# ZhangHaoyang493/News_Recsys

Measured on AMD Instinct MI355X. Metric: impressions/sec at batch 65536 (embedding hot path forward), higher is better.
Workload: dtype f32

## Files before the change

news_recsys_amd/csrc/nrx_interact.hip:

```cpp
#include "nrx_common.h"

namespace {

__global__ __launch_bounds__(NRX_BLOCK) void bag_pool_fwd_kernel(const float* __restrict__ emb, const float* __restrict__ mask,
                                                                 int64_t batch, int L, int D, float* __restrict__ out) {
    const int64_t total = batch * (int64_t)D;
    for (int64_t i = (int64_t)blockIdx.x * NRX_BLOCK + threadIdx.x; i < total; i += (int64_t)gridDim.x * NRX_BLOCK) {
        const int64_t b = i / D;
        const int d = (int)(i - b * D);
        const float* e = emb + (b * L) * (int64_t)D + d;
        float acc = 0.f, den = 0.f;
        if (mask != nullptr) {
            const float* m = mask + b * (int64_t)L;
            for (int l = 0; l < L; ++l) {
#pragma clang fp contract(off)
                const float w = m[l];
                den += w;
                acc += e[(int64_t)l * D] * w;
            }
            out[i] = acc / (den + 1e-8f);
        } else {
            for (int l = 0; l < L; ++l) acc += e[(int64_t)l * D];
            out[i] = acc / (float)L;
        }
    }
}

template <bool VEC>
__global__ __launch_bounds__(NRX_BLOCK) void bag_pool_bwd_kernel(const float* __restrict__ g_out, const float* __restrict__ mask,
                                                                 int64_t batch, int L, int D, float* __restrict__ g_emb) {
    const int lane = threadIdx.x & 63;
    const int64_t wave = (int64_t)blockIdx.x * (NRX_BLOCK / 64) + (threadIdx.x >> 6);
    const int64_t nwaves = (int64_t)gridDim.x * (NRX_BLOCK / 64);
    const int n = L * D;
    for (int64_t b = wave; b < batch; b += nwaves) {
        float den = (float)L;
        if (mask != nullptr) {
            float part = 0.f;
            for (int l = lane; l < L; l += NRX_WAVE) part += mask[b * (int64_t)L + l];
            den = nrx_wave_sum(part) + 1e-8f;
        }
        const float* gb = g_out + b * (int64_t)D;
        const float* mb = mask ? mask + b * (int64_t)L : nullptr;
        float* ob = g_emb + b * (int64_t)n;
        if (VEC) {
            const unsigned q = (unsigned)D >> 2;
            for (unsigned e4 = lane; e4 < (unsigned)n >> 2; e4 += NRX_WAVE) {
                const unsigned l = e4 / q, d = (e4 - l * q) * 4;
                const float4 g = *reinterpret_cast<const float4*>(gb + d);
                const float m = mb ? mb[l] : 1.0f;
                float4 o = make_float4(g.x / den, g.y / den, g.z / den, g.w / den);
                if (mb) o = make_float4(o.x * m, o.y * m, o.z * m, o.w * m);
                *reinterpret_cast<float4*>(ob + (size_t)e4 * 4) = o;
            }
        } else {
            for (int e = lane; e < n; e += NRX_WAVE) {
                const int l = e / D, d = e - l * D;
                const float g = gb[d] / den;
                ob[e] = mb ? g * mb[l] : g;
            }
        }
    }
}

__device__ __forceinline__ float4 ld4(const float* p, int k0, int D, bool vec) {
    float4 v;
    if (vec) {
        v = *reinterpret_cast<const float4*>(p);
    } else {
        v.x = p[0];
        v.y = (k0 + 1 < D) ? p[1] : 0.f;
        v.z = (k0 + 2 < D) ? p[2] : 0.f;
        v.w = (k0 + 3 < D) ? p[3] : 0.f;
    }
    return v;
}

template <int QLOG2>
__global__ __launch_bounds__(NRX_BLOCK) void fm_fwd_kernel(const float* __restrict__ feat, int64_t ld, int F, int D,
                                                           int64_t batch, float* __restrict__ fm_out, bool vec,
                                                           float* __restrict__ sums = nullptr, int64_t sums_ld = 0) {
    constexpr int Q = 1 << QLOG2;
    constexpr int TB = NRX_BLOCK / Q;
    const int q = threadIdx.x & (Q - 1);
    const int64_t b = (int64_t)blockIdx.x * TB + (threadIdx.x >> QLOG2);
    const bool live = b < batch;
    float total = 0.f;
    for (int kc = 0; kc < D; kc += 4 * Q) {
        const int k0 = kc + q * 4;
        float first = 0.f;
        float4 s = make_float4(0.f, 0.f, 0.f, 0.f), sq = s;
        if (live && k0 < D) {
            const float* row = feat + b * ld + k0;
            for (int f = 0; f < F; ++f) {
                float4 v = ld4(row + (int64_t)f * D, k0, D, vec);
                if (k0 == 0) { first += v.x; v.x = 0.f; }
                s.x += v.x; s.y += v.y; s.z += v.z; s.w += v.w;
                sq.x += v.x * v.x; sq.y += v.y * v.y; sq.z += v.z * v.z; sq.w += v.w * v.w;
            }
        }
        total += 0.5f * ((s.x * s.x - sq.x) + (s.y * s.y - sq.y) + (s.z * s.z - sq.z) + (s.w * s.w - sq.w)) + first;
        if (sums != nullptr && live && k0 < D) {
            float* dst = sums + b * sums_ld + k0;
            const float v0 = k0 == 0 ? first : s.x;
            dst[0] = v0;
            if (k0 + 1 < D) dst[1] = s.y;
            if (k0 + 2 < D) dst[2] = s.z;
            if (k0 + 3 < D) dst[3] = s.w;
        }
    }
#pragma unroll
    for (int off = Q / 2; off > 0; off >>= 1) total += __shfl_xor(total, off, 64);
    if (live && q == 0) fm_out[b] = total;
}

template <int QLOG2>
__global__ __launch_bounds__(NRX_BLOCK) void fm_bwd_kernel(const float* __restrict__ feat, int64_t ld, int F, int D, int64_t batch,
                                                           const float* __restrict__ g_fm, const float* g_in, int64_t g_in_ld,
                                                           float* g_feat, int64_t g_ld, bool vec) {
    constexpr int Q = 1 << QLOG2;
    constexpr int TB = NRX_BLOCK / Q;
    constexpr int U = 8;
    const int q = threadIdx.x & (Q - 1);
    const int64_t b = (int64_t)blockIdx.x * TB + (threadIdx.x >> QLOG2);
    if (b >= batch) return;
    const float gl = g_fm[b];
    const bool gvec = vec && (g_ld & 3) == 0 && ((reinterpret_cast<uintptr_t>(g_feat) & 15u) == 0) &&
                      (g_in == nullptr || ((g_in_ld & 3) == 0 && (reinterpret_cast<uintptr_t>(g_in) & 15u) == 0));
    for (int kc = 0; kc < D; kc += 4 * Q) {
        const int k0 = kc + q * 4;
        if (k0 >= D) continue;
        const float* row = feat + b * ld + k0;
        const float* irow = g_in ? g_in + b * g_in_ld + k0 : nullptr;
        float* grow = g_feat + b * g_ld + k0;
        float4 s = make_float4(0.f, 0.f, 0.f, 0.f);
        int f = 0;
        for (; f + U <= F; f += U) {
            float4 v[U];
#pragma unroll
            for (int u = 0; u < U; ++u) v[u] = ld4(row + (int64_t)(f + u) * D, k0, D, vec);
#pragma unroll
            for (int u = 0; u < U; ++u) { s.x += v[u].x; s.y += v[u].y; s.z += v[u].z; s.w += v[u].w; }
        }
        for (; f < F; ++f) {
            const float4 v = ld4(row + (int64_t)f * D, k0, D, vec);
            s.x += v.x; s.y += v.y; s.z += v.z; s.w += v.w;
        }
        f = 0;
        if (gvec && k0 + 4 <= D) {
            for (; f + U <= F; f += U) {
                float4 v[U], up[U];
#pragma unroll
                for (int u = 0; u < U; ++u) {
                    v[u] = ld4(row + (int64_t)(f + u) * D, k0, D, vec);
                    up[u] = irow ? *reinterpret_cast<const float4*>(irow + (int64_t)(f + u) * D) : make_float4(0.f, 0.f, 0.f, 0.f);
                }
#pragma unroll
                for (int u = 0; u < U; ++u) {
                    float4 g = make_float4(gl * (s.x - v[u].x), gl * (s.y - v[u].y), gl * (s.z - v[u].z), gl * (s.w - v[u].w));
                    if (k0 == 0) g.x = gl;
                    *reinterpret_cast<float4*>(grow + (int64_t)(f + u) * D) = make_float4(up[u].x + g.x, up[u].y + g.y, up[u].z + g.z, up[u].w + g.w);
                }
            }
        }
        for (; f < F; ++f) {
            const float4 v = ld4(row + (int64_t)f * D, k0, D, vec);
            float g[4] = {gl * (s.x - v.x), gl * (s.y - v.y), gl * (s.z - v.z), gl * (s.w - v.w)};
            if (k0 == 0) g[0] = gl;
            float* gp = grow + (int64_t)f * D;
            const float* ip = irow ? irow + (int64_t)f * D : nullptr;
#pragma unroll
            for (int j = 0; j < 4; ++j)
                if (k0 + j < D) gp[j] = (ip ? ip[j] : 0.f) + g[j];
        }
    }
}

template <int R, int V>
struct RowRegs {
    float v[R][V];
};

template <int R, int V>
__device__ __forceinline__ void row_load(RowRegs<R, V>& x, const float* p, int D, int lane) {
#pragma unroll
    for (int r = 0; r < R; ++r) {
        const int c = (r * 64 + lane) * V;
        if (V == 4) {
            float4 t = make_float4(0.f, 0.f, 0.f, 0.f);
            if (c < D) t = *reinterpret_cast<const float4*>(p + c);
            x.v[r][0] = t.x; x.v[r][1 % V] = t.y; x.v[r][2 % V] = t.z; x.v[r][3 % V] = t.w;
        } else {
            x.v[r][0] = (c < D) ? p[c] : 0.f;
        }
    }
}

template <int R, int V>
__device__ __forceinline__ void row_store(const RowRegs<R, V>& x, float* p, int D, int lane) {
#pragma unroll
    for (int r = 0; r < R; ++r) {
        const int c = (r * 64 + lane) * V;
        if (c < D) {
            if (V == 4) *reinterpret_cast<float4*>(p + c) = make_float4(x.v[r][0], x.v[r][1 % V], x.v[r][2 % V], x.v[r][3 % V]);
            else p[c] = x.v[r][0];
        }
    }
}

__device__ __forceinline__ float nrx_half_wave_sum(float v, bool upper) {
    v += nrx_dpp<0xB1>(v);
    v += nrx_dpp<0x4E>(v);
    v += nrx_dpp<0x141>(v);
    v += nrx_dpp<0x140>(v);
    const float r0 = __builtin_bit_cast(float, __builtin_amdgcn_readlane(__builtin_bit_cast(int, v), 0));
    const float r1 = __builtin_bit_cast(float, __builtin_amdgcn_readlane(__builtin_bit_cast(int, v), 16));
    const float r2 = __builtin_bit_cast(float, __builtin_amdgcn_readlane(__builtin_bit_cast(int, v), 32));
    const float r3 = __builtin_bit_cast(float, __builtin_amdgcn_readlane(__builtin_bit_cast(int, v), 48));
    return upper ? r2 + r3 : r0 + r1;
}

template <int R, int V, int G = 64>
__device__ __forceinline__ float row_dot(const RowRegs<R, V>& a, const RowRegs<R, V>& b, bool upper = false) {
    float s = 0.f;
#pragma unroll
    for (int r = 0; r < R; ++r)
#pragma unroll
        for (int j = 0; j < V; ++j) s += a.v[r][j] * b.v[r][j];
    return G == 64 ? nrx_wave_sum(s) : nrx_half_wave_sum(s, upper);
}

template <int R, int V, int G = 64>
__global__ __launch_bounds__(NRX_BLOCK) void dcn_v1_fwd_kernel(const float* __restrict__ x, int64_t x_ld, const float* __restrict__ x0p,
                                                               int64_t x0_ld, int64_t batch, int D, int NL,
                                                               const float* __restrict__ w, const float* __restrict__ bvec,
                                                               float* __restrict__ out, int64_t out_ld) {
    extern __shared__ __attribute__((aligned(16))) char smem[];
    float* s_w = reinterpret_cast<float*>(smem);
    const int Dp = (D + 3) & ~3;
    float* s_b = s_w + NL * Dp;
    for (int i = threadIdx.x; i < NL * Dp; i += NRX_BLOCK) {
        const int l = i / Dp, c = i - l * Dp;
        s_w[i] = (c < D) ? w[l * (int64_t)D + c] : 0.f;
        s_b[i] = (c < D) ? bvec[l * (int64_t)D + c] : 0.f;
    }
    __syncthreads();
    constexpr int RPW = 64 / G;
    const int lane = threadIdx.x & (G - 1);
    const bool upper = G == 32 && (threadIdx.x & 32) != 0;
    const int64_t wave = (int64_t)blockIdx.x * (NRX_BLOCK / 64) + (threadIdx.x >> 6);
    const int64_t nwaves = (int64_t)gridDim.x * (NRX_BLOCK / 64);
    for (int64_t r0 = wave * RPW; r0 < batch; r0 += nwaves * RPW) {
        const int64_t rr = r0 + (upper ? 1 : 0);
        const bool live = rr < batch;
        const int64_t row = live ? rr : batch - 1;
        RowRegs<R, V> x0, xl;
        row_load<R, V>(xl, x + row * x_ld, D, lane);
        if (x0p != nullptr) row_load<R, V>(x0, x0p + row * x0_ld, D, lane);
        else x0 = xl;
        for (int l = 0; l < NL; ++l) {
            RowRegs<R, V> wl, bl;
            row_load<R, V>(wl, s_w + l * Dp, Dp, lane);
            row_load<R, V>(bl, s_b + l * Dp, Dp, lane);
            const float s = row_dot<R, V, G>(xl, wl, upper);
#pragma unroll
            for (int r = 0; r < R; ++r)
// ... 386 lines not shown
    const NRX_CONST EmbedDcnArgs* a = nrx_kernarg<EmbedDcnArgs>();
    constexpr int Q = 1 << QLOG2;
    constexpr int TB = NRX_BLOCK / Q;
    extern __shared__ __attribute__((aligned(16))) char smem[];
    const int W = a->width, NL = a->n_layers;
    float4* s_w = reinterpret_cast<float4*>(smem);
    float4* s_b = s_w + NL * (W / 4);
    const int q = threadIdx.x & (Q - 1);
    const int64_t batch = a->batch, stride = (int64_t)gridDim.x * TB;
    int64_t b = (int64_t)blockIdx.x * TB + (threadIdx.x >> QLOG2);
    auto load_ids = [&](int64_t bb, int64_t (&id)[N]) {
        const int64_t bc = bb < batch ? bb : batch - 1;
#pragma unroll
        for (int u = 0; u < N; ++u)
            id[u] = IDX64 ? nrx_gconst<int64_t>(a->index[u])[bc] : (int64_t)nrx_gconst<int32_t>(a->index[u])[bc];
    };
    int64_t id[N];
    load_ids(b, id);
    for (int i = threadIdx.x; i < NL * (W / 4); i += NRX_BLOCK) {
        s_w[i] = reinterpret_cast<const float4*>(a->w)[i];
        s_b[i] = reinterpret_cast<const float4*>(a->b)[i];
    }
    __syncthreads();
    for (; b - (threadIdx.x >> QLOG2) < batch; b += stride) {
        const bool live = b < batch;
        float4 x0[N];
        int bad_feat = -1;
        int64_t bad_id = 0;
#pragma unroll
        for (int u = 0; u < N; ++u) {
            const bool bad = (uint64_t)id[u] >= (uint64_t)a->rows[u];
            bad_feat = bad ? u : bad_feat;
            bad_id = bad ? id[u] : bad_id;
            x0[u] = NT ? nrx_ldg4_nt(a->table[u], (bad ? 0 : id[u]) * Q + q) : nrx_ldg4(a->table[u], (bad ? 0 : id[u]) * Q + q);
        }
        if (bad_feat >= 0 && q == 0 && live) nrx_report_oob(a->status, bad_feat, b, bad_id);
        if (b - (threadIdx.x >> QLOG2) + stride < batch) load_ids(b + stride, id);
        if (EARLY && live) {
            NRX_GLOBAL nrx_f32x4* o = (NRX_GLOBAL nrx_f32x4*)(a->out + b * a->out_ld);
#pragma unroll
            for (int u = 0; u < N; ++u) {
                nrx_f32x4 t;
                t.x = x0[u].x; t.y = x0[u].y; t.z = x0[u].z; t.w = x0[u].w;
                if (STNT) __builtin_nontemporal_store(t, o + u * Q + q);
                else o[u * Q + q] = t;
            }
        }
        float4 xl[N];
#pragma unroll
        for (int u = 0; u < N; ++u) xl[u] = x0[u];
        for (int l = 0; l < NL; ++l) {
            const float4* wl = s_w + l * (W / 4) + q;
            const float4* bl = s_b + l * (W / 4) + q;
            float part = 0.f;
#pragma unroll
            for (int u = 0; u < N; ++u) {
                const float4 wv = wl[u * Q];
                part += xl[u].x * wv.x + xl[u].y * wv.y + xl[u].z * wv.z + xl[u].w * wv.w;
            }
            const float dot = group_sum_dpp<Q>(part);
#pragma unroll
            for (int u = 0; u < N; ++u) {
                const float4 bv = bl[u * Q];
                xl[u].x = x0[u].x * dot + bv.x + xl[u].x;
                xl[u].y = x0[u].y * dot + bv.y + xl[u].y;
                xl[u].z = x0[u].z * dot + bv.z + xl[u].z;
                xl[u].w = x0[u].w * dot + bv.w + xl[u].w;
            }
        }
        if (live) {
            NRX_GLOBAL nrx_f32x4* o = (NRX_GLOBAL nrx_f32x4*)(a->out + b * a->out_ld);
#pragma unroll
            for (int u = EARLY ? N : 0; u < 2 * N; ++u) {
                const float4 v = u < N ? x0[u] : xl[u - N];
                nrx_f32x4 t;
                t.x = v.x; t.y = v.y; t.z = v.z; t.w = v.w;
                NRX_GLOBAL nrx_f32x4* dst = o + (u < N ? 0 : W / 4) + (u < N ? u : u - N) * Q + q;
                if (STNT) __builtin_nontemporal_store(t, dst);
                else *dst = t;
            }
        }
    }
}

int ceil_log2i(int x) {
    int l = 0;
    while ((1 << l) < x) ++l;
    return l;
}

unsigned stream_grid(int64_t items, int per_block) {
    int64_t g = (items + per_block - 1) / per_block;
    const int64_t cap = 256 * 8;
    if (g > cap) g = cap;
    if (g < 1) g = 1;
    return (unsigned)g;
}

#define NRX_QSWITCH(qlog2, ...)               \
    switch (qlog2) {                           \
        case 0: { constexpr int QL = 0; __VA_ARGS__; } break; \
        case 1: { constexpr int QL = 1; __VA_ARGS__; } break; \
        case 2: { constexpr int QL = 2; __VA_ARGS__; } break; \
        case 3: { constexpr int QL = 3; __VA_ARGS__; } break; \
        case 4: { constexpr int QL = 4; __VA_ARGS__; } break; \
        case 5: { constexpr int QL = 5; __VA_ARGS__; } break; \
        default: { constexpr int QL = 6; __VA_ARGS__; } break; \
    }

#define NRX_RSWITCH(R_, V_, ...)                                   \
    if (V_ == 4) {                                                  \
        constexpr int VV = 4;                                       \
        if (R_ <= 1) { constexpr int RR = 1; __VA_ARGS__; }                \
        else if (R_ <= 2) { constexpr int RR = 2; __VA_ARGS__; }           \
        else if (R_ <= 4) { constexpr int RR = 4; __VA_ARGS__; }           \
        else { constexpr int RR = 8; __VA_ARGS__; }                        \
    } else {                                                        \
        constexpr int VV = 1;                                       \
        if (R_ <= 1) { constexpr int RR = 1; __VA_ARGS__; }                \
        else if (R_ <= 2) { constexpr int RR = 2; __VA_ARGS__; }           \
        else if (R_ <= 4) { constexpr int RR = 4; __VA_ARGS__; }           \
        else if (R_ <= 8) { constexpr int RR = 8; __VA_ARGS__; }           \
        else if (R_ <= 16) { constexpr int RR = 16; __VA_ARGS__; }         \
        else { constexpr int RR = 32; __VA_ARGS__; }                       \
    }

}

extern "C" int nrx_bag_pool_fwd(const float* emb, const float* mask, int64_t batch, int32_t bag_len,
                                int32_t dim, float* out, void* stream) {
    NRX_TRACE();
    NRX_REQUIRE(emb && out && batch >= 0 && bag_len >= 1 && dim >= 1, "nrx_bag_pool_fwd: bad argument");
    if (batch == 0) return NRX_OK;
    hipLaunchKernelGGL(bag_pool_fwd_kernel, dim3(stream_grid(batch * dim, NRX_BLOCK)), dim3(NRX_BLOCK), 0,
                       reinterpret_cast<hipStream_t>(stream), emb, mask, batch, bag_len, dim, out);
    NRX_LAUNCH_CHECK("nrx_bag_pool_fwd");
    return NRX_OK;
}

extern "C" int nrx_bag_pool_bwd(const float* g_out, const float* mask, int64_t batch, int32_t bag_len,
                                int32_t dim, float* g_emb, void* stream) {
    NRX_TRACE();
    NRX_REQUIRE(g_out && g_emb && batch >= 0 && bag_len >= 1 && dim >= 1, "nrx_bag_pool_bwd: bad argument");
    if (batch == 0) return NRX_OK;
    const bool vec = (dim & 3) == 0 && nrx_aligned16(g_out) && nrx_aligned16(g_emb);
    if (vec) hipLaunchKernelGGL(bag_pool_bwd_kernel<true>, dim3(stream_grid(batch, NRX_BLOCK / 64)), dim3(NRX_BLOCK), 0,
                                reinterpret_cast<hipStream_t>(stream), g_out, mask, batch, bag_len, dim, g_emb);
    else hipLaunchKernelGGL(bag_pool_bwd_kernel<false>, dim3(stream_grid(batch, NRX_BLOCK / 64)), dim3(NRX_BLOCK), 0,
                            reinterpret_cast<hipStream_t>(stream), g_out, mask, batch, bag_len, dim, g_emb);
    NRX_LAUNCH_CHECK("nrx_bag_pool_bwd");
    return NRX_OK;
}

extern "C" int nrx_fm_fwd(const float* feat, int64_t ld, int32_t n_fields, int32_t dim, int64_t batch,
                          float* fm_out, void* stream) {
    NRX_TRACE();
    NRX_REQUIRE(feat && fm_out && n_fields >= 1 && dim >= 1 && batch >= 0 && ld >= (int64_t)n_fields * dim,
                "nrx_fm_fwd: bad argument");
    if (batch == 0) return NRX_OK;
    int ql = ceil_log2i((dim + 3) / 4);
    if (ql > 6) ql = 6;
    const bool vec = (dim & 3) == 0 && (ld & 3) == 0 && nrx_aligned16(feat);
    const int tb = NRX_BLOCK >> ql;
    const unsigned grid = (unsigned)((batch + tb - 1) / tb);
    NRX_QSWITCH(ql, { hipLaunchKernelGGL((fm_fwd_kernel<QL>), dim3(grid), dim3(NRX_BLOCK), 0, reinterpret_cast<hipStream_t>(stream),
                                         feat, ld, n_fields, dim, batch, fm_out, vec); });
    NRX_LAUNCH_CHECK("nrx_fm_fwd");
    return NRX_OK;
}

extern "C" int nrx_fm_fwd_train(const float* feat, int64_t ld, int32_t n_fields, int32_t dim, int64_t batch,
                                float* fm_out, float* fm_sums, int64_t sums_ld, void* stream) {
    NRX_TRACE();
    NRX_REQUIRE(feat && fm_out && fm_sums && n_fields >= 1 && dim >= 1 && batch >= 0 && ld >= (int64_t)n_fields * dim && sums_ld >= dim,
                "nrx_fm_fwd_train: bad argument");
    if (batch == 0) return NRX_OK;
    int ql = ceil_log2i((dim + 3) / 4);
    if (ql > 6) ql = 6;
    const bool vec = (dim & 3) == 0 && (ld & 3) == 0 && nrx_aligned16(feat);
    const int tb = NRX_BLOCK >> ql;
    const unsigned grid = (unsigned)((batch + tb - 1) / tb);
    NRX_QSWITCH(ql, { hipLaunchKernelGGL((fm_fwd_kernel<QL>), dim3(grid), dim3(NRX_BLOCK), 0, reinterpret_cast<hipStream_t>(stream),
                                         feat, ld, n_fields, dim, batch, fm_out, vec, fm_sums, sums_ld); });
    NRX_LAUNCH_CHECK("nrx_fm_fwd_train");
    return NRX_OK;
}

extern "C" int nrx_fm_bwd(const float* feat, int64_t ld, int32_t n_fields, int32_t dim, int64_t batch,
                          const float* g_fm, const float* g_in, int64_t g_in_ld, float* g_feat, int64_t g_ld, void* stream) {
    NRX_TRACE();
    NRX_REQUIRE(feat && g_fm && g_feat && n_fields >= 1 && dim >= 1 && batch >= 0, "nrx_fm_bwd: bad argument");
    if (batch == 0) return NRX_OK;
    int ql = ceil_log2i((dim + 3) / 4);
    if (ql > 6) ql = 6;
    const bool vec = (dim & 3) == 0 && (ld & 3) == 0 && nrx_aligned16(feat);
    const int tb = NRX_BLOCK >> ql;
    const unsigned grid = (unsigned)((batch + tb - 1) / tb);
    NRX_QSWITCH(ql, { hipLaunchKernelGGL((fm_bwd_kernel<QL>), dim3(grid), dim3(NRX_BLOCK), 0, reinterpret_cast<hipStream_t>(stream),
                                         feat, ld, n_fields, dim, batch, g_fm, g_in, g_in_ld, g_feat, g_ld, vec); });
    NRX_LAUNCH_CHECK("nrx_fm_bwd");
    return NRX_OK;
}

namespace {
constexpr int FH_BLOCKS = 64;
__global__ __launch_bounds__(NRX_BLOCK) void fm_head_fwd_kernel(const float* __restrict__ logit, const float* __restrict__ bias, float* __restrict__ out,
                                                                int64_t batch) {
    const float b = bias != nullptr ? bias[0] : 0.f;
    for (int64_t i = (int64_t)blockIdx.x * NRX_BLOCK + threadIdx.x; i < batch; i += (int64_t)gridDim.x * NRX_BLOCK) {
        const float x = b + logit[i];
        out[i] = 1.0f / (1.0f + expf(-x));
    }
}
__global__ __launch_bounds__(NRX_BLOCK) void fm_head_bwd_kernel(const float* __restrict__ g_out, int64_t g_stride, const float* __restrict__ out,
                                                                float* __restrict__ g_logit, float* __restrict__ g_bias, uint32_t* __restrict__ state,
                                                                int64_t batch) {
    __shared__ float s_w[NRX_BLOCK / 64];
    __shared__ uint32_t s_last;
    const int64_t chunk = (batch + gridDim.x - 1) / gridDim.x;
    const int64_t lo = (int64_t)blockIdx.x * chunk, hi = lo + chunk < batch ? lo + chunk : batch;
    float acc = 0.f;
    for (int64_t i = lo + threadIdx.x; i < hi; i += NRX_BLOCK) {
        const float p = out[i];
        const float g = g_out[i * g_stride] * (p * (1.0f - p));
        g_logit[i] = g;
        acc += g;
    }
    if (g_bias == nullptr) return;
    acc = nrx_wave_sum(acc);
    if ((threadIdx.x & 63) == 0) s_w[threadIdx.x >> 6] = acc;
    __syncthreads();
    float* partial = reinterpret_cast<float*>(state + 8);
    if (threadIdx.x == 0) {
        partial[blockIdx.x] = (s_w[0] + s_w[1]) + (s_w[2] + s_w[3]);
        __threadfence();
        s_last = atomicAdd(&state[0], 1u) == gridDim.x - 1 ? 1u : 0u;
    }
    __syncthreads();
    if (s_last && threadIdx.x < 64) {
        __threadfence();
        float v = (int)threadIdx.x < (int)gridDim.x ? __hip_atomic_load(&partial[threadIdx.x], __ATOMIC_RELAXED, __HIP_MEMORY_SCOPE_AGENT) : 0.f;
        v = nrx_wave_sum(v);
        if (threadIdx.x == 0) {
            g_bias[0] = v;
            state[0] = 0;
        }
    }
}
}

extern "C" int nrx_fm_head_fwd(const float* logit, const float* bias, float* out, int64_t batch, void* stream) {
    NRX_TRACE();
    NRX_REQUIRE(logit && out && batch >= 0, "nrx_fm_head_fwd: bad argument");
    if (batch == 0) return NRX_OK;
    const int64_t g = (batch + NRX_BLOCK - 1) / NRX_BLOCK;
    hipLaunchKernelGGL(fm_head_fwd_kernel, dim3((unsigned)(g < 1024 ? g : 1024)), dim3(NRX_BLOCK), 0, reinterpret_cast<hipStream_t>(stream), logit, bias, out, batch);
    NRX_LAUNCH_CHECK("nrx_fm_head_fwd");
    return NRX_OK;
}

extern "C" int64_t nrx_fm_head_state_bytes(void) { return 32 + FH_BLOCKS * 4; }

extern "C" int nrx_fm_head_bwd(const float* g_out, int64_t g_stride, const float* out, float* g_logit, float* g_bias, void* state, int64_t batch,
                               void* stream) {
    NRX_TRACE();
    NRX_REQUIRE(g_out && out && g_logit && batch >= 0 && (g_stride == 0 || g_stride == 1), "nrx_fm_head_bwd: bad argument");
    NRX_REQUIRE(g_bias == nullptr || state != nullptr, "nrx_fm_head_bwd: the bias gradient needs the state words (nrx_fm_head_state_bytes, zero before the first use)");
    if (batch == 0) {
        if (g_bias != nullptr && nrx_zero_async(g_bias, 4, reinterpret_cast<hipStream_t>(stream)) != NRX_OK) return NRX_ERR_LAUNCH;
        return NRX_OK;
    }
    const int64_t g = (batch + 1023) / 1024;
    hipLaunchKernelGGL(fm_head_bwd_kernel, dim3((unsigned)(g < FH_BLOCKS ? g : FH_BLOCKS)), dim3(NRX_BLOCK), 0, reinterpret_cast<hipStream_t>(stream), g_out, g_stride,
                       out, g_logit, g_bias, reinterpret_cast<uint32_t*>(state), batch);
    NRX_LAUNCH_CHECK("nrx_fm_head_bwd");
    return NRX_OK;
}

extern "C" int nrx_dcn_v1_fwd(const float* x, int64_t x_ld, const float* x0, int64_t x0_ld, int64_t batch, int32_t dim,
                              int32_t n_layers, const float* w, const float* b, float* out, int64_t out_ld, void* stream) {
    NRX_TRACE();
    NRX_REQUIRE(x && out && batch >= 0 && dim >= 1, "nrx_dcn_v1_fwd: bad argument");
    if (x0 == x && x0_ld == x_ld) x0 = nullptr;
    NRX_REQUIRE(n_layers >= 0 && n_layers <= NRX_MAX_DCN_LAYERS, "nrx_dcn_v1_fwd: n_layers must be in [0, %d]", NRX_MAX_DCN_LAYERS);
    NRX_REQUIRE(n_layers == 0 || (w && b), "nrx_dcn_v1_fwd: null cross weights");
    NRX_REQUIRE(dim <= 2048, "nrx_dcn_v1_fwd: dim %d > 2048 unsupported", dim);
    if (batch == 0) return NRX_OK;
    const bool vec = (dim & 3) == 0 && (x_ld & 3) == 0 && (out_ld & 3) == 0 && nrx_aligned16(x) && nrx_aligned16(out) &&
                     (x0 == nullptr || ((x0_ld & 3) == 0 && nrx_aligned16(x0)));
    const int V = vec ? 4 : 1;
    const int R = (dim + 64 * V - 1) / (64 * V);
    const size_t smem = (size_t)2 * n_layers * ((dim + 3) & ~3) * sizeof(float);
    NRX_REQUIRE(smem <= 64 * 1024, "nrx_dcn_v1_fwd: n_layers*dim too large for the LDS stage");
    if (vec && dim <= 128) {
        const unsigned grid2 = stream_grid((batch + 1) / 2, NRX_BLOCK / 64);
        hipLaunchKernelGGL((dcn_v1_fwd_kernel<1, 4, 32>), dim3(grid2), dim3(NRX_BLOCK), smem, reinterpret_cast<hipStream_t>(stream),
                           x, x_ld, x0, x0_ld, batch, dim, n_layers, w, b, out, out_ld);
        NRX_LAUNCH_CHECK("nrx_dcn_v1_fwd(half-wave rows)");
        return NRX_OK;
    }
    const unsigned grid = stream_grid(batch, NRX_BLOCK / 64);
    NRX_RSWITCH(R, V, { hipLaunchKernelGGL((dcn_v1_fwd_kernel<RR, VV>), dim3(grid), dim3(NRX_BLOCK), smem, reinterpret_cast<hipStream_t>(stream),
                                           x, x_ld, x0, x0_ld, batch, dim, n_layers, w, b, out, out_ld); });
    NRX_LAUNCH_CHECK("nrx_dcn_v1_fwd");
    return NRX_OK;
}

constexpr int DCN_V1_MAX_BLOCKS = 1024;
static int dcn_v1_bwd_impl(const float* x, int64_t x_ld, const float* x0, int64_t x0_ld, int64_t batch, int32_t dim,
                           int32_t n_layers, const float* w, const float* b, const float* g_out, int64_t g_out_ld,
                           float* g_x, int64_t g_x_ld, float* g_x0, int64_t g_x0_ld, float* g_w_user, float* g_b_user, void* stream,
                           float* ordered_ws, unsigned* grid_out) {
    const int ordered = ordered_ws != nullptr ? 1 : 0;
    float* g_w = ordered ? ordered_ws : g_w_user;
    float* g_b = ordered ? ordered_ws + (size_t)DCN_V1_MAX_BLOCKS * (n_layers > 0 ? n_layers : 1) * dim : g_b_user;
    unsigned last_grid = 0;
    struct GridOut { unsigned* p; unsigned* v; ~GridOut() { if (p) *p = *v; } } grid_guard{grid_out, &last_grid};
    NRX_REQUIRE(x && g_out && g_x && batch >= 0 && dim >= 1, "nrx_dcn_v1_bwd: bad argument");
    if (x0 == x && x0_ld == x_ld && g_x0 == nullptr) x0 = nullptr;
    NRX_REQUIRE((x0 == nullptr) == (g_x0 == nullptr), "nrx_dcn_v1_bwd: x0 and g_x0 go together (both null: x0 is x, one gradient)");
    NRX_REQUIRE(n_layers >= 0 && n_layers <= NRX_MAX_DCN_LAYERS, "nrx_dcn_v1_bwd: n_layers must be in [0, %d]", NRX_MAX_DCN_LAYERS);
    NRX_REQUIRE(n_layers == 0 || (w && b && g_w && g_b), "nrx_dcn_v1_bwd: null cross weights");
    if (ordered && n_layers > 0) {
        const size_t Dp_ = (size_t)((dim + 3) & ~3);
        const bool vec_ = (dim & 3) == 0;
        if (((size_t)4 * n_layers + (size_t)(vec_ && dim <= 128 ? 8 : 4) * n_layers * 2) * Dp_ * sizeof(float) > 128 * 1024 &&
            !(n_layers <= 4 && (dim + 64 * (vec_ ? 4 : 1) - 1) / (64 * (vec_ ? 4 : 1)) <= 2)) {
            nrx_set_error("nrx_dcn_v1_bwd_ordered: n_layers * dim too large for the ordered mode");
            return NRX_ERR_UNSUPPORTED;
// ... 259 lines not shown
```

news_recsys_amd/csrc/nrx_route_feat.hip:

```cpp
#include <cstring>

#include "nrx_common.h"

namespace {

constexpr int RF_THREADS = 256;
#ifndef NRX_RF_ROUNDS
#define NRX_RF_ROUNDS 16
#endif
constexpr int RF_ROUNDS = NRX_RF_ROUNDS;
constexpr int RF_TILE = RF_THREADS * RF_ROUNDS;
constexpr int RF_WAVES = RF_THREADS / 64;
constexpr int RF_MAX_WORLD = 64;

struct RouteFeatArgs {
    const void* ids[NRX_MAX_FEATURES];
    int64_t batch;
    int64_t capf;
    int32_t n_feats, world, idx64, tiles;
    int32_t* send_ids;
    int32_t* send_pos;
    int32_t* slot;
    int64_t* counts;
    int64_t* overflow;
// ... 330 lines not shown
    }
    uint32_t opn = 0, cls = 0;
    if constexpr (RUNS) {
        uint16_t* s_smp = reinterpret_cast<uint16_t*>(s_aux);
        __syncthreads();
        if (tid == 0) {
            int run = 0;
            for (int o = 0; o < W; ++o) { s_pref[o] = run; run += s_tot[o]; }
        }
        __syncthreads();
#pragma unroll
        for (int j = 0; j < RF_ROUNDS; ++j) rank[j] += owner[j] >= 0 ? s_cell[j * RF_WAVES + wid][owner[j]] : 0;
#pragma unroll
        for (int j = 0; j < RF_ROUNDS; ++j) {
            if (owner[j] < 0) continue;
            s_smp[s_pref[owner[j]] + rank[j]] = (uint16_t)local_sample(j);
        }
        __syncthreads();
#pragma unroll
        for (int j = 0; j < RF_ROUNDS; ++j) {
            if (owner[j] < 0) continue;
            const int o = owner[j];
            const int at = s_pref[o] + rank[j];
            const uint16_t me = (uint16_t)local_sample(j);
            if (rank[j] == 0 || s_smp[at - 1] != me) opn |= 1u << j;
            if (rank[j] == s_tot[o] - 1 || s_smp[at + 1] != me) cls |= 1u << j;
        }
    }
    auto poll = [&](const unsigned long long* p) -> int {
        unsigned long long v;
        do { v = __hip_atomic_load(p, __ATOMIC_RELAXED, __HIP_MEMORY_SCOPE_AGENT); } while ((uint32_t)(v >> 32) != mark);
        return (int)(uint32_t)v;
    };
    auto tiles_before_in_group = [&](int x, int* dst) {
        const int g0 = x / RB_GROUP, nt = (x - g0 * RB_GROUP) * W;
        for (int j = tid; j < nt; j += RF_THREADS) atomicAdd(&dst[j % W], poll(&a->agg[(int64_t)g0 * RB_GROUP * W + j]));
    };
    auto groups_before = [&](int x, int* dst) {
        const int ng = (x / RB_GROUP) * W;
        for (int j = tid; j < ng; j += RF_THREADS) atomicAdd(&dst[j % W], poll(&a->gagg[j]));
    };
    const bool last_of_feat = w + 1 == a->tile0[f + 1];
#ifndef NRX_RB_NO_CHAIN
    tiles_before_in_group(w, s_base);
    __syncthreads();
    if ((w % RB_GROUP) == RB_GROUP - 1 && tid < W)
        __hip_atomic_store(&a->gagg[(int64_t)(w / RB_GROUP) * W + tid], ((unsigned long long)mark << 32) | (unsigned)(s_base[tid] + s_tot[tid]), __ATOMIC_RELAXED,
                           __HIP_MEMORY_SCOPE_AGENT);
    groups_before(w, s_base);
    if (last_of_feat) {
        tiles_before_in_group(a->tile0[f], s_feat);
        groups_before(a->tile0[f], s_feat);
    }
#endif
    __syncthreads();
    const int64_t cap = a->cap, B = a->batch;
    const int L = a->bag_len[f];
    const uint64_t magic_l = a->magic_len[f];
    const int32_t tag0 = (int32_t)(f * B);
    const int64_t ntag_r = (int64_t)n * B;
#pragma unroll
    for (int j = 0; j < RF_ROUNDS; ++j) {
        if (owner[j] < 0) continue;
        const int o = owner[j];
        const int64_t i = i0 + j * RF_THREADS + tid;
        const int pt = RUNS ? rank[j] : s_cell[j * RF_WAVES + wid][o] + rank[j];
        const int64_t k = (int64_t)s_base[o] + pt;
        const int32_t smp = RUNS ? (int32_t)smp0 + local_sample(j) : (L == 1 ? (int32_t)i : (int32_t)__umul64hi((uint64_t)i, magic_l));
#ifdef NRX_RB_NO_STORE
        if (k < 0) {
#else
        if (k < cap) {
#endif
            const int64_t d = (int64_t)o * cap + k;
            a->send_rows[d] = val[j];
            if (!RUNS) a->send_tag[d] = tag0 + smp;
            a->send_w[d] = wt[j];
        }
        if (RUNS && ((opn | cls) >> j) & 1u) {
            int32_t* r = a->send_run + ((int64_t)o * ntag_r + tag0 + smp) * 2;
            if ((opn >> j) & 1u) r[0] = (int32_t)(k < cap ? k : cap);
            if ((cls >> j) & 1u) r[1] = (int32_t)(k + 1 < cap ? k + 1 : cap);
        }
    }
    if (last_of_feat && tid < W) a->counts2d[(int64_t)tid * n + f] = (int64_t)s_base[tid] + s_tot[tid] - s_feat[tid];
    if (w == T - 1 && tid == 0) {
        long long worst = 0;
        for (int o = 0; o < W; ++o) {
            const long long c = (long long)s_base[o] + s_tot[o];
            worst = c > worst ? c : worst;
        }
        atomicMax(reinterpret_cast<long long*>(a->overflow), worst);
    }
    __syncthreads();
    if (w == T - 1 && tid == 0) {
        __hip_atomic_store(&a->ctl[2], mark, __ATOMIC_RELAXED, __HIP_MEMORY_SCOPE_AGENT);
        __hip_atomic_store(&a->ctl[0], 0u, __ATOMIC_RELAXED, __HIP_MEMORY_SCOPE_AGENT);
    }
}

__global__ __launch_bounds__(NRX_BLOCK) void inbox_transpose_kernel(const int32_t* __restrict__ a_in, int32_t* __restrict__ a_out,
                                                                   const int32_t* __restrict__ b_in, int32_t* __restrict__ b_out, int world, int n,
                                                                   int64_t capf) {
    const int64_t total = (int64_t)world * n * capf;
    for (int64_t i = ((int64_t)blockIdx.x * NRX_BLOCK + threadIdx.x) * 4; i < total; i += (int64_t)gridDim.x * NRX_BLOCK * 4) {
        const int64_t run = i / capf, k = i - run * capf;
        const int s = (int)(run / n), f = (int)(run - (int64_t)s * n);
        const int64_t o = ((int64_t)f * world + s) * capf + k;
        typedef int nrx_i32x4t __attribute__((ext_vector_type(4)));
        *reinterpret_cast<nrx_i32x4t*>(a_out + o) = *reinterpret_cast<const nrx_i32x4t*>(a_in + i);
        if (b_in != nullptr) *reinterpret_cast<nrx_i32x4t*>(b_out + o) = *reinterpret_cast<const nrx_i32x4t*>(b_in + i);
    }
}

#ifndef NRX_GP_R
#define NRX_GP_R 8
#endif
constexpr int GP_R = NRX_GP_R;
struct GatherPlaceArgs {
    const float* table[NRX_MAX_FEATURES];
    int64_t rows[NRX_MAX_FEATURES];
    int32_t col[NRX_MAX_FEATURES];
    float* peer[RF_MAX_WORLD];
    const int32_t* oid;
    const int32_t* opos;
    int64_t bp, capf, ld, out_rows;
    int32_t n, world;
    int32_t* status;
};
static_assert(sizeof(GatherPlaceArgs) <= 3584, "kernarg budget");

typedef unsigned nrx_gp_u32x2 __attribute__((ext_vector_type(2)));
template <int QLOG2, typename TS = float>
__global__ __launch_bounds__(NRX_BLOCK) void gather_place_feat_kernel(const GatherPlaceArgs args_in_kernarg) {
    const NRX_CONST GatherPlaceArgs* a = nrx_kernarg<GatherPlaceArgs>();
    constexpr int Q = 1 << QLOG2, TB = NRX_BLOCK / Q;
    const int q = threadIdx.x & (Q - 1);
    const int64_t bp = a->bp;
    const int n = a->n;
    for (int64_t b = (int64_t)blockIdx.x * TB + (threadIdx.x >> QLOG2); b < bp; b += (int64_t)gridDim.x * TB) {
        const int s = (int)(b / a->capf);
        float* __restrict__ out = a->peer[s];
        auto fetch = [&](int f0, int32_t* id, int32_t* pos) {
#pragma unroll
            for (int r = 0; r < GP_R; ++r) {
                const int f = f0 + r < n ? f0 + r : n - 1;
                id[r] = nrx_gconst<int32_t>(a->oid)[(int64_t)f * bp + b];
                pos[r] = nrx_gconst<int32_t>(a->opos)[(int64_t)f * bp + b];
            }
        };
        auto process = [&](int f0, const int32_t* id, int32_t* pos) {
            float4 v[GP_R];
            [[maybe_unused]] nrx_gp_u32x2 raw[GP_R];
            [[maybe_unused]] bool use[GP_R];
#pragma unroll
            for (int r = 0; r < GP_R; ++r) {
                const int f = f0 + r < n ? f0 + r : n - 1;
                v[r] = make_float4(0.f, 0.f, 0.f, 0.f);
                if constexpr (sizeof(TS) == 2) {
                    const uint64_t tb = reinterpret_cast<uint64_t>(a->table[f]);
                    const uint32_t tb_lo = __builtin_amdgcn_readfirstlane((uint32_t)tb), tb_hi = __builtin_amdgcn_readfirstlane((uint32_t)(tb >> 32));
                    const uint32_t nr = __builtin_amdgcn_readfirstlane((uint32_t)(a->rows[f] > 0x7fffffff ? 0x7fffffff : a->rows[f]));
                    const NRX_GLOBAL nrx_gp_u32x2* base = (const NRX_GLOBAL nrx_gp_u32x2*)(((uint64_t)tb_hi << 32) | tb_lo);
                    use[r] = f0 + r < n && pos[r] >= 0 && id[r] > 0 && (uint32_t)id[r] < nr;
                    raw[r] = __builtin_nontemporal_load(base + ((int64_t)(use[r] ? id[r] : 0) * Q + q));
                }
                if (f0 + r >= n || pos[r] < 0) { pos[r] = -1; continue; }
                if (id[r] < 0 || (int64_t)id[r] >= a->rows[f]) {
                    if (q == 0) nrx_report_oob(a->status, f, b, id[r]);
                    continue;
                }
                if constexpr (sizeof(TS) != 2) {
                    if (id[r] != 0) v[r] = nrx_ldg4_nt(a->table[f], (int64_t)id[r] * Q + q);
                }
            }
#pragma unroll
            for (int r = 0; r < GP_R; ++r) {
                if (pos[r] < 0) continue;
                const int f = f0 + r;
                if ((int64_t)pos[r] >= a->out_rows) {
                    if (q == 0) nrx_report_oob(a->status, f, b, pos[r]);
                    continue;
                }
                if constexpr (sizeof(TS) == 2) {
                    if (use[r]) v[r] = nrx_bf16x4_to_f32(raw[r].x, raw[r].y);
                }
                nrx_stg4(out, ((int64_t)pos[r] * a->ld + a->col[f]) / 4 + q, v[r]);
            }
        };
        int32_t ida[GP_R], posa[GP_R], idb[GP_R], posb[GP_R];
        fetch(0, ida, posa);
        for (int f0 = 0; f0 < n; f0 += 2 * GP_R) {
            if (f0 + GP_R < n) fetch(f0 + GP_R, idb, posb);
            process(f0, ida, posa);
            if (f0 + GP_R >= n) break;
            if (f0 + 2 * GP_R < n) fetch(f0 + 2 * GP_R, ida, posa);
            process(f0 + GP_R, idb, posb);
        }
    }
}

__global__ __launch_bounds__(NRX_BLOCK) void shard_dest_combine_kernel(const int32_t* __restrict__ slot, const int32_t* __restrict__ dest_req, int n, int64_t batch,
                                                                      int64_t capf, int64_t recv_row0, int rank, int shift, int32_t* __restrict__ out) {
    const int f = blockIdx.y;
    const uint32_t un = (uint32_t)n, ucapf = (uint32_t)capf;
    for (int64_t b = (int64_t)blockIdx.x * NRX_BLOCK + threadIdx.x; b < batch; b += (int64_t)gridDim.x * NRX_BLOCK) {
        const int64_t p = (int64_t)f * batch + b;
        const int32_t sl = slot[p];
        int32_t r = -1;
        if (sl >= 0) {
            const uint32_t ok = (uint32_t)sl / un, o = ok / ucapf, k = ok - o * ucapf;
            const int32_t d = dest_req[((int64_t)o * n + f) * capf + k];
            const int64_t row = d >= 0 ? (int64_t)d : recv_row0 + ((int64_t)rank * capf + k) * n + f;
            r = (int32_t)(((int64_t)o << shift) | row);
        }
        out[p] = r;
    }
}

bool all_resident(const void* kernel, int64_t blocks) {
    static thread_local const void* cached_k[4] = {nullptr, nullptr, nullptr, nullptr};
    static thread_local int64_t cached_cap[4] = {0, 0, 0, 0};
    int64_t capacity = -1;
    for (int i = 0; i < 4; ++i)
        if (cached_k[i] == kernel) capacity = cached_cap[i];
    if (capacity < 0) {
        int per_cu = 0, dev = 0, cus = 0;
        if (hipOccupancyMaxActiveBlocksPerMultiprocessor(&per_cu, kernel, RF_THREADS, 0) != hipSuccess || hipGetDevice(&dev) != hipSuccess ||
            hipDeviceGetAttribute(&cus, hipDeviceAttributeMultiprocessorCount, dev) != hipSuccess)
            return false;
        capacity = (int64_t)per_cu * cus;
        for (int i = 0; i < 4; ++i)
            if (cached_k[i] == nullptr) { cached_k[i] = kernel; cached_cap[i] = capacity; break; }
    }
    return blocks <= capacity;
}

}

extern "C" int nrx_shard_dest_combine(const int32_t* slot, const int32_t* dest_req, int32_t n_feats, int64_t batch, int64_t capf, int64_t recv_row0,
                                      int32_t rank, int32_t world, int32_t shift, int32_t* dest_out, void* stream) {
    NRX_TRACE();
    NRX_REQUIRE(slot && dest_req && dest_out && n_feats >= 1 && batch >= 0 && capf >= 1 && rank >= 0 && rank < world, "nrx_shard_dest_combine: bad argument");
    NRX_REQUIRE(shift >= 1 && shift <= 30 && (int64_t)world <= (1ll << (31 - shift)) && recv_row0 + (int64_t)world * capf * n_feats <= (1ll << shift),
                "nrx_shard_dest_combine: (owner << shift) | row must fit 31 bits");
    if (batch == 0) return NRX_OK;
    NRX_REQUIRE(capf < 0x7fffffffLL && n_feats <= NRX_MAX_FEATURES, "nrx_shard_dest_combine: capf must fit 31 bits, n_feats <= %d", NRX_MAX_FEATURES);
    int64_t blocks = (batch + NRX_BLOCK - 1) / NRX_BLOCK;
    if (blocks > 1024) blocks = 1024;
    hipLaunchKernelGGL(shard_dest_combine_kernel, dim3((unsigned)blocks, (unsigned)n_feats), dim3(NRX_BLOCK), 0, reinterpret_cast<hipStream_t>(stream), slot, dest_req, (int)n_feats,
                       batch, capf, recv_row0, (int)rank, (int)shift, dest_out);
    NRX_LAUNCH_CHECK("nrx_shard_dest_combine");
    return NRX_OK;
}

namespace {
template <typename TS>
int gather_place_feat_launch(const char* who, const void* const* tables, const int64_t* table_rows, const int32_t* feat_col, int32_t n_feats, int32_t world,
                                     int64_t capf, const int32_t* owner_ids, const int32_t* owner_pos, int32_t dim, float* const* peer_out,
                                     int64_t out_ld, int64_t out_rows, int32_t* status, void* stream) {
    NRX_REQUIRE(tables && table_rows && feat_col && owner_ids && owner_pos && peer_out, "%s: null argument", who);
    NRX_REQUIRE(n_feats >= 1 && n_feats <= NRX_MAX_FEATURES && world >= 1 && world <= RF_MAX_WORLD && capf >= 1, "%s: bad sizes", who);
    if (!(dim == 16 || dim == 32 || dim == 64 || dim == 128 || dim == 256) || (out_ld & 3) != 0) {
        nrx_set_error("%s: dim must be 16 / 32 / 64 / 128 / 256 and out_ld a multiple of 4", who);
        return NRX_ERR_UNSUPPORTED;
    }
    GatherPlaceArgs a;
    memset(&a, 0, sizeof(a));
    for (int i = 0; i < n_feats; ++i) {
        NRX_REQUIRE(tables[i] != nullptr && (reinterpret_cast<uintptr_t>(tables[i]) & (sizeof(TS) == 2 ? 7u : 15u)) == 0 && (feat_col[i] & 3) == 0,
                    "%s: feature %d: aligned table and column", who, i);
        NRX_REQUIRE(sizeof(TS) != 2 || table_rows[i] >= 1, "%s: feature %d: a bf16 arena has at least its dummy row", who, i);
        a.table[i] = reinterpret_cast<const float*>(tables[i]);
        a.rows[i] = table_rows[i];
        a.col[i] = feat_col[i];
    }
    for (int s = 0; s < world; ++s) {
        NRX_REQUIRE(peer_out[s] != nullptr && nrx_aligned16(peer_out[s]), "%s: peer %d: null / unaligned buffer", who, s);
        a.peer[s] = peer_out[s];
    }
    a.oid = owner_ids;
    a.opos = owner_pos;
    a.bp = (int64_t)world * capf;
    a.capf = capf;
    a.ld = out_ld;
    a.out_rows = out_rows;
    a.n = n_feats;
    a.world = world;
    a.status = status;
    const int ql = dim == 16 ? 2 : dim == 32 ? 3 : dim == 64 ? 4 : dim == 128 ? 5 : 6;
    const int64_t tb = NRX_BLOCK >> ql;
    int64_t blocks = (a.bp + tb - 1) / tb;
    if (blocks > 8192) blocks = 8192;
    hipStream_t st = reinterpret_cast<hipStream_t>(stream);
    if (ql == 2) hipLaunchKernelGGL((gather_place_feat_kernel<2, TS>), dim3((unsigned)blocks), dim3(NRX_BLOCK), 0, st, a);
    else if (ql == 3) hipLaunchKernelGGL((gather_place_feat_kernel<3, TS>), dim3((unsigned)blocks), dim3(NRX_BLOCK), 0, st, a);
    else if (ql == 4) hipLaunchKernelGGL((gather_place_feat_kernel<4, TS>), dim3((unsigned)blocks), dim3(NRX_BLOCK), 0, st, a);
    else if (ql == 5) hipLaunchKernelGGL((gather_place_feat_kernel<5, TS>), dim3((unsigned)blocks), dim3(NRX_BLOCK), 0, st, a);
    else hipLaunchKernelGGL((gather_place_feat_kernel<6, TS>), dim3((unsigned)blocks), dim3(NRX_BLOCK), 0, st, a);
    NRX_LAUNCH_CHECK(who);
    return NRX_OK;
}
}

extern "C" int nrx_gather_place_feat(const float* const* tables, const int64_t* table_rows, const int32_t* feat_col, int32_t n_feats, int32_t world,
                                     int64_t capf, const int32_t* owner_ids, const int32_t* owner_pos, int32_t dim, float* const* peer_out,
                                     int64_t out_ld, int64_t out_rows, int32_t* status, void* stream) {
    NRX_TRACE();
    return gather_place_feat_launch<float>("nrx_gather_place_feat", reinterpret_cast<const void* const*>(tables), table_rows, feat_col, n_feats, world, capf,
                                           owner_ids, owner_pos, dim, peer_out, out_ld, out_rows, status, stream);
}

extern "C" int nrx_gather_place_feat_bf16(const uint16_t* const* tables, const int64_t* table_rows, const int32_t* feat_col, int32_t n_feats, int32_t world,
                                          int64_t capf, const int32_t* owner_ids, const int32_t* owner_pos, int32_t dim, float* const* peer_out,
                                          int64_t out_ld, int64_t out_rows, int32_t* status, void* stream) {
    NRX_TRACE();
    return gather_place_feat_launch<uint16_t>("nrx_gather_place_feat_bf16", reinterpret_cast<const void* const*>(tables), table_rows, feat_col, n_feats, world,
                                              capf, owner_ids, owner_pos, dim, peer_out, out_ld, out_rows, status, stream);
}

extern "C" int64_t nrx_route_feat_state_bytes(int32_t n_feats, int64_t batch, int32_t world) {
    if (n_feats < 1 || n_feats > NRX_MAX_FEATURES || batch < 0 || world < 1 || world > RF_MAX_WORLD) return -1;
    const int64_t tiles = (batch + RF_TILE - 1) / RF_TILE;
    return 512 + (int64_t)n_feats * (tiles > 0 ? tiles : 1) * world * 8;
}

extern "C" int nrx_route_feat(const void* const* ids, int32_t n_feats, int64_t batch, int32_t index_bits, int32_t world, int64_t capf,
                              int32_t* send_ids, int32_t* send_pos, int32_t* slot, int64_t* counts, int64_t* overflow, void* state, void* stream) {
    NRX_TRACE();
    NRX_REQUIRE(ids != nullptr && n_feats >= 1 && n_feats <= NRX_MAX_FEATURES, "nrx_route_feat: n_feats must be in [1, %d]", NRX_MAX_FEATURES);
    NRX_REQUIRE(world >= 1 && world <= RF_MAX_WORLD, "nrx_route_feat: world must be in [1, %d]", RF_MAX_WORLD);
    NRX_REQUIRE(index_bits == 32 || index_bits == 64, "nrx_route_feat: index_bits must be 32 or 64");
    NRX_REQUIRE(batch >= 0 && batch < 0x7fffffffLL && capf >= 1, "nrx_route_feat: bad batch / capf");
    NRX_REQUIRE((int64_t)world * capf * n_feats < 0x7fffffffLL, "nrx_route_feat: world * capf * n_feats must stay below 2^31 (slot is int32)");
    NRX_REQUIRE(send_ids && slot && counts && overflow && state, "nrx_route_feat: null buffer");
    if (batch == 0) return NRX_OK;
    RouteFeatArgs a;
    memset(&a, 0, sizeof(a));
    for (int i = 0; i < n_feats; ++i) {
        NRX_REQUIRE(ids[i] != nullptr, "nrx_route_feat: feature %d: null ids", i);
        a.ids[i] = ids[i];
    }
    a.batch = batch;
    a.capf = capf;
    a.n_feats = n_feats;
    a.world = world;
    a.idx64 = index_bits == 64;
    a.tiles = (int32_t)((batch + RF_TILE - 1) / RF_TILE);
    a.send_ids = send_ids;
    a.send_pos = send_pos;
    a.slot = slot;
    a.counts = counts;
    a.overflow = overflow;
    a.ctl = reinterpret_cast<uint32_t*>(state);
    a.agg = reinterpret_cast<unsigned long long*>(reinterpret_cast<char*>(state) + 512);
    a.use_ticket = world > 1 && !all_resident(reinterpret_cast<const void*>(route_feat_kernel), (int64_t)n_feats * a.tiles);
    hipLaunchKernelGGL(route_feat_kernel, dim3((unsigned)(n_feats * a.tiles)), dim3(RF_THREADS), 0, reinterpret_cast<hipStream_t>(stream), a);
    NRX_LAUNCH_CHECK("nrx_route_feat");
    return NRX_OK;
}

extern "C" int64_t nrx_route_bags_one_state_bytes(const int32_t* bag_lens, int32_t n_feats, int64_t batch, int32_t world) {
    if (bag_lens == nullptr || n_feats < 1 || n_feats > NRX_MAX_FEATURES || batch < 0 || world < 1 || world > RF_MAX_WORLD) return -1;
    int64_t tiles = 0;
    for (int f = 0; f < n_feats; ++f) tiles += (batch * bag_lens[f] + RF_TILE - 1) / RF_TILE;
    return 64 + ((tiles > 0 ? tiles : 1) + tiles / RB_GROUP + 1) * world * 8;
}

extern "C" int nrx_route_bags_one(const void* const* ids, const float* const* weights, const int32_t* bag_lens, int32_t n_feats, int32_t index_bits,
                                  int64_t batch, int32_t world, int64_t cap, int32_t* send_rows, int32_t* send_tag, float* send_w, int64_t* counts2d,
                                  int64_t* overflow, void* state, void* stream) {
    NRX_TRACE();
    NRX_REQUIRE(ids && bag_lens && n_feats >= 1 && n_feats <= NRX_MAX_FEATURES, "nrx_route_bags_one: n_feats must be in [1, %d]", NRX_MAX_FEATURES);
    NRX_REQUIRE(index_bits == 32 || index_bits == 64, "nrx_route_bags_one: index_bits must be 32 or 64");
    NRX_REQUIRE(world >= 1 && world <= RF_MAX_WORLD && cap >= 1 && cap * world <= 0x7fffffffLL && batch >= 0, "nrx_route_bags_one: bad world / cap / batch");
    NRX_REQUIRE((int64_t)n_feats * batch <= 0x7fffffffLL, "nrx_route_bags_one: n_feats * batch must fit 31 bits");
    NRX_REQUIRE(send_rows && send_tag && send_w && counts2d && overflow && state, "nrx_route_bags_one: null buffer");
    RouteBagsArgs a;
    memset(&a, 0, sizeof(a));
    int64_t tiles = 0, total = 0;
    for (int f = 0; f < n_feats; ++f) {
        NRX_REQUIRE(bag_lens[f] >= 1 && (batch == 0 || ids[f] != nullptr), "nrx_route_bags_one: feature %d: bad ids / bag_len", f);
        a.ids[f] = ids[f];
        a.weight[f] = weights ? weights[f] : nullptr;
        a.bag_len[f] = bag_lens[f];
        a.magic_len[f] = bag_lens[f] > 1 ? ~0ull / (uint64_t)bag_lens[f] + 1 : 0;
        a.tile0[f] = (int32_t)tiles;
        tiles += (batch * bag_lens[f] + RF_TILE - 1) / RF_TILE;
        total += batch * bag_lens[f];
    }
    a.tile0[n_feats] = (int32_t)tiles;
    a.magic_world = world > 1 ? ~0ull / (uint64_t)world + 1 : 0;
    NRX_REQUIRE(total <= 0x7fffffffLL && tiles < (1 << 24), "nrx_route_bags_one: too many ids for one exchange");
    if (tiles == 0) return NRX_OK;
    a.batch = batch;
    a.cap = cap;
    a.n_feats = n_feats;
    a.world = world;
    a.idx64 = index_bits == 64;
    a.tiles = (int32_t)tiles;
    a.send_rows = send_rows;
    a.send_tag = send_tag;
    a.send_w = send_w;
    a.counts2d = counts2d;
    a.overflow = overflow;
    a.ctl = reinterpret_cast<uint32_t*>(state);
    a.agg = reinterpret_cast<unsigned long long*>(reinterpret_cast<char*>(state) + 64);
    a.gagg = a.agg + tiles * world;
    a.use_ticket = !all_resident(reinterpret_cast<const void*>(route_bags_one_kernel<false>), tiles);
    hipLaunchKernelGGL(route_bags_one_kernel<false>, dim3((unsigned)tiles), dim3(RF_THREADS), 0, reinterpret_cast<hipStream_t>(stream), a);
    NRX_LAUNCH_CHECK("nrx_route_bags_one");
    return NRX_OK;
}

static bool route_bags_runs_ok(const int32_t* bag_lens, int32_t n_feats, int32_t world) {
    for (int f = 0; f < n_feats; ++f)
        if (bag_lens[f] < 1 || bag_lens[f] > RF_TILE || (int64_t)(RF_TILE / bag_lens[f]) * world > RF_TILE) return false;
    return true;
}

extern "C" int64_t nrx_route_bags_runs_state_bytes(const int32_t* bag_lens, int32_t n_feats, int64_t batch, int32_t world) {
    if (bag_lens == nullptr || n_feats < 1 || n_feats > NRX_MAX_FEATURES || batch < 0 || world < 1 || world > RF_MAX_WORLD) return -1;
    if (!route_bags_runs_ok(bag_lens, n_feats, world)) return 0;
    int64_t tiles = 0;
    for (int f = 0; f < n_feats; ++f) {
// ... 74 lines not shown
```

Baseline: 1.054 billion.

## Add dim-16 FM forward kernel on cache lines and unconditional fp32 gather loads

Adds a specialised FM forward kernel for dim 16. Eight lanes cover a 128-byte line pair, splitting fields by parity and exchanging values via DPP, with U=7 unrolled loads kept in flight. It is used by default when alignment allows and can be turned off with NRX_FM_LINES=0. Separately, the fp32 gather-place path now issues its table loads unconditionally, with a uniform base via readfirstlane and row 0 as the fallback, then masks the result afterwards. This hoists loads out of the branchy checks to raise memory-level parallelism. The cost is extra clamped loads of the dummy row and a new requirement that fp32 tables have at least one row.

```diff
diff --git a/news_recsys_amd/csrc/nrx_interact.hip b/news_recsys_amd/csrc/nrx_interact.hip
--- a/news_recsys_amd/csrc/nrx_interact.hip
+++ b/news_recsys_amd/csrc/nrx_interact.hip
@@ -112,6 +112,57 @@
 #pragma unroll
     for (int off = Q / 2; off > 0; off >>= 1) total += __shfl_xor(total, off, 64);
     if (live && q == 0) fm_out[b] = total;
+}
+
+constexpr int FM_LINES_U = 7;
+__global__ __launch_bounds__(NRX_BLOCK) void fm_fwd_lines_kernel(const float* __restrict__ feat, int64_t ld, int F, int64_t batch,
+                                                                 float* __restrict__ fm_out, float* __restrict__ sums, int64_t sums_ld) {
+    constexpr int U = FM_LINES_U, TB = NRX_BLOCK / 8;
+    const int q = threadIdx.x & 3, par = (threadIdx.x >> 2) & 1;
+    const int64_t b = (int64_t)blockIdx.x * TB + (threadIdx.x >> 3);
+    const bool live = b < batch;
+    const int np = (F + 1) >> 1;
+    const float* row = feat + (live ? b : batch - 1) * ld + q * 4;
+    float first = 0.f;
+    float4 s = make_float4(0.f, 0.f, 0.f, 0.f), sq = s;
+    auto add = [&](float4 v) {
+        if (q == 0) { first += v.x; v.x = 0.f; }
+        s.x += v.x; s.y += v.y; s.z += v.z; s.w += v.w;
+        sq.x = __builtin_fmaf(v.x, v.x, sq.x); sq.y = __builtin_fmaf(v.y, v.y, sq.y);
+        sq.z = __builtin_fmaf(v.z, v.z, sq.z); sq.w = __builtin_fmaf(v.w, v.w, sq.w);
+    };
+    for (int j0 = 0; j0 < np; j0 += U) {
+        float4 v[U];
+#pragma unroll
+        for (int u = 0; u < U; ++u) {
+            const int j = j0 + u < np ? j0 + u : np - 1;
+            const int f = 2 * j + par;
+            v[u] = nrx_ldg4(row, (int64_t)(f < F ? f : F - 1) * 4);
+        }
+#pragma unroll
+        for (int u = 0; u < U; ++u) {
+            const int j = j0 + u;
+            const float4 o = make_float4(nrx_dpp<0x104>(v[u].x), nrx_dpp<0x104>(v[u].y), nrx_dpp<0x104>(v[u].z), nrx_dpp<0x104>(v[u].w));
+            if (j < np) add(v[u]);
+            if (2 * j + 1 < F) add(o);
+        }
+    }
+    float total = 0.f;
+    {
+#pragma clang fp contract(off)
+        const float dx = __builtin_fmaf(s.x, s.x, -sq.x), dy = __builtin_fmaf(s.y, s.y, -sq.y);
+        const float pz = s.z * s.z, pw = s.w * s.w;
+        const float dz = pz - sq.z, dw = pw - sq.w;
+        const float sum = ((dx + dy) + dz) + dw;
+        total += __builtin_fmaf(0.5f, sum, first);
+    }
+    if (sums != nullptr && live && par == 0) {
+        if (q == 0) s.x = first;
+        nrx_stg4(sums, (b * sums_ld) / 4 + q, s);
+    }
+    total += __shfl_xor(total, 2, 64);
+    total += __shfl_xor(total, 1, 64);
+    if (live && (threadIdx.x & 7) == 0) fm_out[b] = total;
 }
 
 template <int QLOG2>
@@ -804,12 +855,31 @@
     return NRX_OK;
 }
 
+namespace {
+bool fm_lines_ok(const float* feat, int64_t ld, int dim, const float* sums, int64_t sums_ld) {
+    const char* e = getenv("NRX_FM_LINES");
+    if (e && atoi(e) == 0) return false;
+    return dim == 16 && (reinterpret_cast<uintptr_t>(feat) & 127u) == 0 && (ld & 31) == 0 &&
+           (sums == nullptr || (nrx_aligned16(sums) && (sums_ld & 3) == 0));
+}
+void fm_lines_launch(const float* feat, int64_t ld, int F, int64_t batch, float* fm_out, float* sums, int64_t sums_ld, void* stream) {
+    constexpr int tb = NRX_BLOCK / 8;
+    hipLaunchKernelGGL(fm_fwd_lines_kernel, dim3((unsigned)((batch + tb - 1) / tb)), dim3(NRX_BLOCK), 0, reinterpret_cast<hipStream_t>(stream), feat, ld, F,
+                       batch, fm_out, sums, sums_ld);
+}
+}
+
 extern "C" int nrx_fm_fwd(const float* feat, int64_t ld, int32_t n_fields, int32_t dim, int64_t batch,
                           float* fm_out, void* stream) {
     NRX_TRACE();
     NRX_REQUIRE(feat && fm_out && n_fields >= 1 && dim >= 1 && batch >= 0 && ld >= (int64_t)n_fields * dim,
                 "nrx_fm_fwd: bad argument");
     if (batch == 0) return NRX_OK;
+    if (fm_lines_ok(feat, ld, dim, nullptr, 0)) {
+        fm_lines_launch(feat, ld, n_fields, batch, fm_out, nullptr, 0, stream);
+        NRX_LAUNCH_CHECK("nrx_fm_fwd");
+        return NRX_OK;
+    }
     int ql = ceil_log2i((dim + 3) / 4);
     if (ql > 6) ql = 6;
     const bool vec = (dim & 3) == 0 && (ld & 3) == 0 && nrx_aligned16(feat);
@@ -827,6 +897,11 @@
     NRX_REQUIRE(feat && fm_out && fm_sums && n_fields >= 1 && dim >= 1 && batch >= 0 && ld >= (int64_t)n_fields * dim && sums_ld >= dim,
                 "nrx_fm_fwd_train: bad argument");
     if (batch == 0) return NRX_OK;
+    if (fm_lines_ok(feat, ld, dim, fm_sums, sums_ld)) {
+        fm_lines_launch(feat, ld, n_fields, batch, fm_out, fm_sums, sums_ld, stream);
+        NRX_LAUNCH_CHECK("nrx_fm_fwd_train");
+        return NRX_OK;
+    }
     int ql = ceil_log2i((dim + 3) / 4);
     if (ql > 6) ql = 6;
     const bool vec = (dim & 3) == 0 && (ld & 3) == 0 && nrx_aligned16(feat);
diff --git a/news_recsys_amd/csrc/nrx_route_feat.hip b/news_recsys_amd/csrc/nrx_route_feat.hip
--- a/news_recsys_amd/csrc/nrx_route_feat.hip
+++ b/news_recsys_amd/csrc/nrx_route_feat.hip
@@ -506,26 +506,28 @@
         auto process = [&](int f0, const int32_t* id, int32_t* pos) {
             float4 v[GP_R];
             [[maybe_unused]] nrx_gp_u32x2 raw[GP_R];
-            [[maybe_unused]] bool use[GP_R];
+            bool use[GP_R];
 #pragma unroll
             for (int r = 0; r < GP_R; ++r) {
                 const int f = f0 + r < n ? f0 + r : n - 1;
                 v[r] = make_float4(0.f, 0.f, 0.f, 0.f);
+                const uint64_t tb = reinterpret_cast<uint64_t>(a->table[f]);
+                const uint32_t tb_lo = __builtin_amdgcn_readfirstlane((uint32_t)tb), tb_hi = __builtin_amdgcn_readfirstlane((uint32_t)(tb >> 32));
                 if constexpr (sizeof(TS) == 2) {
-                    const uint64_t tb = reinterpret_cast<uint64_t>(a->table[f]);
-                    const uint32_t tb_lo = __builtin_amdgcn_readfirstlane((uint32_t)tb), tb_hi = __builtin_amdgcn_readfirstlane((uint32_t)(tb >> 32));
                     const uint32_t nr = __builtin_amdgcn_readfirstlane((uint32_t)(a->rows[f] > 0x7fffffff ? 0x7fffffff : a->rows[f]));
                     const NRX_GLOBAL nrx_gp_u32x2* base = (const NRX_GLOBAL nrx_gp_u32x2*)(((uint64_t)tb_hi << 32) | tb_lo);
                     use[r] = f0 + r < n && pos[r] >= 0 && id[r] > 0 && (uint32_t)id[r] < nr;
                     raw[r] = __builtin_nontemporal_load(base + ((int64_t)(use[r] ? id[r] : 0) * Q + q));
+                } else {
+                    const uint32_t nr = __builtin_amdgcn_readfirstlane(a->rows[f] > 0x7fffffff ? 0x80000000u : (uint32_t)(a->rows[f] < 0 ? 0 : a->rows[f]));
+                    const float* base = reinterpret_cast<const float*>(((uint64_t)tb_hi << 32) | tb_lo);
+                    use[r] = f0 + r < n && pos[r] >= 0 && id[r] > 0 && (uint32_t)id[r] < nr;
+                    v[r] = nrx_ldg4_nt(base, (int64_t)(use[r] ? id[r] : 0) * Q + q);
                 }
                 if (f0 + r >= n || pos[r] < 0) { pos[r] = -1; continue; }
                 if (id[r] < 0 || (int64_t)id[r] >= a->rows[f]) {
                     if (q == 0) nrx_report_oob(a->status, f, b, id[r]);
                     continue;
-                }
-                if constexpr (sizeof(TS) != 2) {
-                    if (id[r] != 0) v[r] = nrx_ldg4_nt(a->table[f], (int64_t)id[r] * Q + q);
                 }
             }
 #pragma unroll
@@ -538,6 +540,8 @@
                 }
                 if constexpr (sizeof(TS) == 2) {
                     if (use[r]) v[r] = nrx_bf16x4_to_f32(raw[r].x, raw[r].y);
+                } else {
+                    if (!use[r]) v[r] = make_float4(0.f, 0.f, 0.f, 0.f);
                 }
                 nrx_stg4(out, ((int64_t)pos[r] * a->ld + a->col[f]) / 4 + q, v[r]);
             }
@@ -624,7 +628,7 @@
     for (int i = 0; i < n_feats; ++i) {
         NRX_REQUIRE(tables[i] != nullptr && (reinterpret_cast<uintptr_t>(tables[i]) & (sizeof(TS) == 2 ? 7u : 15u)) == 0 && (feat_col[i] & 3) == 0,
                     "%s: feature %d: aligned table and column", who, i);
-        NRX_REQUIRE(sizeof(TS) != 2 || table_rows[i] >= 1, "%s: feature %d: a bf16 arena has at least its dummy row", who, i);
+        NRX_REQUIRE(table_rows[i] >= 1, "%s: feature %d: an arena has at least its dummy row", who, i);
         a.table[i] = reinterpret_cast<const float*>(tables[i]);
         a.rows[i] = table_rows[i];
         a.col[i] = feat_col[i];
```

Result: no change. 1.050 billion (-0.4%).
